# mikwieczorek/centroids-reid

Measured on AMD Instinct MI355X. Metric: train_images_per_sec, higher is better.
Workload: dtype bf16; 1 GPU; ResNet50 256x128 CTL training step: fwd+bwd, centroid-triplet + center + xent, Adam + center SGD (BASELINE configs[1]); P=16, K=4, global_batch=64, num_classes=751, parallelism=single

## Files before the change

centroids-reid_amd/csrc/conv_igemm.hip:

```cpp
#include "conv_common.hpp"
#include <type_traits>
#include "wgrad_reduce.hpp"
#include "tune.hpp"
#include <stdlib.h>

bool wgrad_make_reduce_job(const creid_conv_desc* d, int dtype, const void* ws, size_t ws_bytes, float* dw, int accumulate,
                           WRedJob& j);
int wgrad_reduce_job_launch(const WRedJob& j, hipStream_t s);
int launch_stream1x1(int M, int K, int N, const void* src, const void* wgt, void* out, float* bn_part, hipStream_t s);
int launch_stream2(int M, int K, int N, const void* src, const void* wgt, void* out, float* bn_part, const void* add_src,
                   const float* epi_scale, const float* epi_shift, int epi_relu, int bn_cap, int dtype, hipStream_t s);
int launch_conv3x3_c64(int M, int H, int Wd, const void* src, const void* wgt, void* out, float* bn_part, const float* epi_scale,
                       const float* epi_shift, int epi_relu, int dtype, hipStream_t s);
int launch_igemm_pp(const IGemmGeom& g, const void* src, const void* wgt, void* out, const void* add_src, float* bn_part,
                    int variant, int dtype, hipStream_t s);

__device__ __attribute__((aligned(128))) unsigned g_zero_page[32];

template <int BN>
__global__ __launch_bounds__(256, BN == 128 ? 1 : 2) void igemm_bf16_kernel(IGemmGeom g, const unsigned short* __restrict__ src,
                                                         const unsigned short* __restrict__ wgt,
                                                         unsigned short* __restrict__ out,
                                                         const unsigned short* __restrict__ add_src,
                                                         float* __restrict__ bn_part, int tiles_n) {
  constexpr int BK = 64, TNW = BN / 64, NB = BN / 32;
  constexpr int CP = BN + 8;
  constexpr int LDS_ELEMS = (128 * BK + BN * BK) > (128 * CP) ? (128 * BK + BN * BK) : (128 * CP);
  __shared__ __attribute__((aligned(16))) unsigned short smem[LDS_ELEMS];
  unsigned short* As = smem;
  unsigned short* Bs = smem + 128 * BK;
  const int tid = threadIdx.x, lane = tid & 63, wave = tid >> 6;
  const int wm = wave >> 1, wn = wave & 1;
  const int bid = xcd_remap(blockIdx.x, gridDim.x);
  const int tile_m = bid / tiles_n, tile_n = bid % tiles_n;
  const int row0 = tile_m * 128, col0 = tile_n * BN;
  const int span_mask = (1 << g.log2span) - 1;
  const bool tap_uniform = g.log2span >= 6;

  const int lrow = tid >> 3, lch = tid & 7;
  int oy[4], ox[4], bpix[4], soff[4];
  bool vm[4];
#pragma unroll
  for (int i = 0; i < 4; ++i) {
    const int r = lrow + 32 * i, m = row0 + r;
    vm[i] = m < g.M;
    const int mm = vm[i] ? m : 0;
    int b, rem;
    fast_divmod(mm, g.OH * g.OW, g.inv_ohow, b, rem);
    fast_divmod(rem, g.OW, g.inv_ow, oy[i], ox[i]);
    bpix[i] = b * g.SH * g.SW;
    soff[i] = r * BK + ((lch ^ ((r >> 1) & 7)) << 3);
  }
  const unsigned short* wp[NB];
#pragma unroll
  for (int i = 0; i < NB; ++i) wp[i] = wgt + (int64_t)(col0 + lrow + 32 * i) * g.K + 8 * lch;

  const unsigned short* aptr[4];
  int amul[4];
  int cur_tap = -1;
  const unsigned short* zpage = reinterpret_cast<const unsigned short*>(g_zero_page) + 8 * lch;
  auto set_tap = [&](int tap) {
    const int r = tap / g.kw, s = tap - r * g.kw;
#pragma unroll
    for (int i = 0; i < 4; ++i) {
      int iy, ix;
      const bool ok = vm[i] && igemm_src_pixel(g, oy[i], ox[i], r, s, iy, ix);
      aptr[i] = ok ? src + (int64_t)(bpix[i] + iy * g.SW + ix) * g.pitch + 8 * lch : zpage;
      amul[i] = ok ? 1 : 0;
    }
  };
  typedef unsigned u32x4 __attribute__((ext_vector_type(4)));
  struct Stage { u32x4 a0, a1, a2, a3, b0, b1, b2, b3; };
  Stage st0, st1, st2;
  const u32x4 zero4 = {0u, 0u, 0u, 0u};
#define IGEMM_LDA(I_, DST, C_) DST = *reinterpret_cast<const u32x4*>(aptr[I_] + (C_) * amul[I_])
#define IGEMM_LDA_G(I_, DST, R_, S_, C_)                                                                \
  do {                                                                                                  \
    int iy, ix;                                                                                         \
    if (vm[I_] && igemm_src_pixel(g, oy[I_], ox[I_], R_, S_, iy, ix))                                   \
      DST = *reinterpret_cast<const u32x4*>(src + (int64_t)(bpix[I_] + iy * g.SW + ix) * g.pitch + (C_)); \
    else                                                                                                \
      DST = zero4;                                                                                      \
  } while (0)
#define IGEMM_GLOAD(T_, ST)                                                                             \
  do {                                                                                                  \
    const int t_ = (T_);                                                                                \
    if (tap_uniform) {                                                                                  \
      const int tap_ = (t_ * BK) >> g.log2span;                                                         \
      if (tap_ != cur_tap) { set_tap(tap_); cur_tap = tap_; }                                           \
      const int c_ = (t_ * BK) & span_mask;                                                             \
      IGEMM_LDA(0, ST.a0, c_); IGEMM_LDA(1, ST.a1, c_); IGEMM_LDA(2, ST.a2, c_); IGEMM_LDA(3, ST.a3, c_); \
    } else {                                                                                            \
      const int kk_ = t_ * BK + 8 * lch;                                                                \
      const int tap_ = kk_ >> g.log2span, c_ = kk_ & span_mask;                                         \
      const int r_ = tap_ / g.kw, s_ = tap_ - r_ * g.kw;                                                \
      IGEMM_LDA_G(0, ST.a0, r_, s_, c_); IGEMM_LDA_G(1, ST.a1, r_, s_, c_);                             \
      IGEMM_LDA_G(2, ST.a2, r_, s_, c_); IGEMM_LDA_G(3, ST.a3, r_, s_, c_);                             \
    }                                                                                                   \
    ST.b0 = *reinterpret_cast<const u32x4*>(wp[0] + t_ * BK);                                           \
    ST.b1 = *reinterpret_cast<const u32x4*>(wp[1] + t_ * BK);                                           \
    if constexpr (NB == 4) {                                                                            \
      ST.b2 = *reinterpret_cast<const u32x4*>(wp[2] + t_ * BK);                                         \
      ST.b3 = *reinterpret_cast<const u32x4*>(wp[3] + t_ * BK);                                         \
    }                                                                                                   \
  } while (0)
#define IGEMM_LSTORE(ST)                                                                                \
  do {                                                                                                  \
    *reinterpret_cast<u32x4*>(&As[soff[0]]) = ST.a0; *reinterpret_cast<u32x4*>(&As[soff[1]]) = ST.a1;   \
    *reinterpret_cast<u32x4*>(&As[soff[2]]) = ST.a2; *reinterpret_cast<u32x4*>(&As[soff[3]]) = ST.a3;   \
    *reinterpret_cast<u32x4*>(&Bs[soff[0]]) = ST.b0; *reinterpret_cast<u32x4*>(&Bs[soff[1]]) = ST.b1;   \
    if constexpr (NB == 4) {                                                                            \
      *reinterpret_cast<u32x4*>(&Bs[soff[2]]) = ST.b2; *reinterpret_cast<u32x4*>(&Bs[soff[3]]) = ST.b3; \
    }                                                                                                   \
  } while (0)

  f32x16 acc[2][TNW];
#pragma unroll
  for (int i = 0; i < 2; ++i)
#pragma unroll
    for (int j = 0; j < TNW; ++j)
#pragma unroll
      for (int r = 0; r < 16; ++r) acc[i][j][r] = 0.f;

  const int nk = g.K / BK;
  const int l31 = lane & 31, kh = lane >> 5;
  auto compute = [&]() {
#pragma unroll
    for (int kk = 0; kk < 4; ++kk) {
      const int ch = 2 * kk + kh;
      s16x8 a[2], b[TNW];
#pragma unroll
      for (int i = 0; i < 2; ++i) {
        const int r = wm * 64 + i * 32 + l31;
        a[i] = *reinterpret_cast<const s16x8*>(&As[r * BK + ((ch ^ ((r >> 1) & 7)) << 3)]);
      }
#pragma unroll
      for (int j = 0; j < TNW; ++j) {
        const int c = wn * (BN / 2) + j * 32 + l31;
        b[j] = *reinterpret_cast<const s16x8*>(&Bs[c * BK + ((ch ^ ((c >> 1) & 7)) << 3)]);
      }
#pragma unroll
      for (int i = 0; i < 2; ++i)
#pragma unroll
        for (int j = 0; j < TNW; ++j)
          acc[i][j] = __builtin_amdgcn_mfma_f32_32x32x16_bf16(__builtin_bit_cast(bf16x8, a[i]),
                                                              __builtin_bit_cast(bf16x8, b[j]), acc[i][j], 0, 0, 0);
    }
  };
  const int last = nk - 1;
  IGEMM_GLOAD(0, st0);
  IGEMM_GLOAD(min(1, last), st1);
  IGEMM_GLOAD(min(2, last), st2);
  const int nk3 = nk - nk % 3;
  int t = 0;
  for (; t < nk3; t += 3) {
    __syncthreads();
    IGEMM_LSTORE(st0);
    __syncthreads();
    IGEMM_GLOAD(min(t + 3, last), st0);
    compute();
    __syncthreads();
    IGEMM_LSTORE(st1);
    __syncthreads();
    IGEMM_GLOAD(min(t + 4, last), st1);
    compute();
    __syncthreads();
    IGEMM_LSTORE(st2);
    __syncthreads();
    IGEMM_GLOAD(min(t + 5, last), st2);
    compute();
  }
  for (; t < nk; ++t) {
    __syncthreads();
    IGEMM_LSTORE(st0);
    __syncthreads();
    st0 = st1;
    compute();
  }
#undef IGEMM_GLOAD
#undef IGEMM_LSTORE
#undef IGEMM_LDA
#undef IGEMM_LDA_G
  __syncthreads();

  float s1v[TNW], s2v[TNW];
#pragma unroll
  for (int j = 0; j < TNW; ++j) {
    const int cl = wn * (BN / 2) + j * 32 + l31;
    float s1 = 0.f, s2 = 0.f;
#pragma unroll
    for (int i = 0; i < 2; ++i) {
#pragma unroll
      for (int r = 0; r < 16; ++r) {
        const int rl = wm * 64 + i * 32 + (r & 3) + 8 * (r >> 2) + 4 * kh;
        const float v = acc[i][j][r];
        s1 += v; s2 = fmaf(v, v, s2);
        smem[rl * CP + cl] = f32_to_bf16_bits(v);
      }
    }
    s1 += __shfl_xor(s1, 32, 64); s2 += __shfl_xor(s2, 32, 64);
    s1v[j] = s1; s2v[j] = s2;
  }
  __syncthreads();
  constexpr int CPR = BN / 8;
#pragma unroll
  for (int i = 0; i < (128 * CPR) / 256; ++i) {
    const int id = tid + 256 * i, rl = id / CPR, ch = id - rl * CPR;
    const int rr = row0 + rl;
    if (rr < g.M) {
      uint4 v = *reinterpret_cast<const uint4*>(&smem[rl * CP + ch * 8]);
      const int64_t off = (int64_t)rr * g.N + col0 + ch * 8;
      if (add_src) {
        const uint4 a = *reinterpret_cast<const uint4*>(add_src + off);
        unsigned* vw = &v.x; const unsigned* aw = &a.x;
#pragma unroll
        for (int q = 0; q < 4; ++q) {
          const float lo = __uint_as_float(vw[q] << 16) + __uint_as_float(aw[q] << 16);
          const float hi = __uint_as_float(vw[q] & 0xffff0000u) + __uint_as_float(aw[q] & 0xffff0000u);
          vw[q] = (unsigned)f32_to_bf16_bits(lo) | ((unsigned)f32_to_bf16_bits(hi) << 16);
        }
      }
      *reinterpret_cast<uint4*>(out + off) = v;
    }
  }
  if (bn_part) {
    __syncthreads();
    float* red = reinterpret_cast<float*>(smem);
#pragma unroll
    for (int j = 0; j < TNW; ++j) {
      const int cl = wn * (BN / 2) + j * 32 + l31;
      if (kh == 0) { red[(wm * 2 + 0) * BN + cl] = s1v[j]; red[(wm * 2 + 1) * BN + cl] = s2v[j]; }
    }
    __syncthreads();
    for (int i = tid; i < 2 * BN; i += 256) {
      const int which = i / BN, cl = i - which * BN;
      bn_part[((int64_t)tile_m * 2 + which) * g.N + col0 + cl] = red[(0 * 2 + which) * BN + cl] + red[(1 * 2 + which) * BN + cl];
    }
  }
}

template <int N> __device__ __forceinline__ void wait_vm() { asm volatile("s_waitcnt vmcnt(%0)" ::"n"(N) : "memory"); }

template <int BN, int NS, typename ET = Bf16T>
__global__ __launch_bounds__(256, (NS * (128 + BN) * 128 <= 80 * 1024) ? 2 : 1) void igemm_bf16_dma_kernel(IGemmGeom g, const unsigned short* __restrict__ src,
                                                                 const unsigned short* __restrict__ wgt,
                                                                 unsigned short* __restrict__ out,
                                                                 const unsigned short* __restrict__ add_src,
                                                                 float* __restrict__ bn_part, int tiles_n,
                                                                 BnRedArgs bnred) {
  constexpr int BK = 64, TNW = BN / 64, NBI = BN / 32;
  constexpr int CPT = 128 + 4;
  constexpr int TILE_A = 128 * BK, TILE_B = BN * BK, STAGE = TILE_A + TILE_B;
  constexpr int LDS_ELEMS = (NS * STAGE) > (BN * CPT) ? (NS * STAGE) : (BN * CPT);
  constexpr int LPT = 4 + NBI;
  static_assert((NS - 2) * LPT <= 63, "vmcnt is a 6-bit counter");
  __shared__ __attribute__((aligned(1024))) unsigned short smem[LDS_ELEMS];
  const int tid = threadIdx.x, lane = tid & 63, wave = tid >> 6;
  const int wm = wave >> 1, wn = wave & 1;
  const int bid = xcd_remap(blockIdx.x, gridDim.x);
  const int tile_m = bid / tiles_n, tile_n = bid % tiles_n;
  const int row0 = tile_m * 128, col0 = tile_n * BN;
  const int span_mask = (1 << g.log2span) - 1;

  const int lr8 = lane >> 3, lcp = lane & 7;
  int oy[4], ox[4], bpix[4], gch[4];
  bool vm[4];
#pragma unroll
  for (int i = 0; i < 4; ++i) {
    const int r = (i * 4 + wave) * 8 + lr8, m = row0 + r;
    vm[i] = m < g.M;
    const int mm = vm[i] ? m : 0;
    int b, rem;
    fast_divmod(mm, g.OH * g.OW, g.inv_ohow, b, rem);
    fast_divmod(rem, g.OW, g.inv_ow, oy[i], ox[i]);
    bpix[i] = b * g.SH * g.SW;
    gch[i] = (lcp ^ ((r >> 1) & 7)) << 3;
  }
  const unsigned short* wp[NBI];
#pragma unroll
  for (int i = 0; i < NBI; ++i) {
    const int r = (i * 4 + wave) * 8 + lr8;
    wp[i] = wgt + (int64_t)(col0 + r) * g.K + ((lcp ^ ((r >> 1) & 7)) << 3);
  }
  const unsigned short* aptr[4];
  int amul[4];
  int cur_tap = -1, cur_r = 0, cur_s = -1;
  const unsigned short* zpage = reinterpret_cast<const unsigned short*>(g_zero_page);
  auto set_tap = [&]() {
    if (++cur_s == g.kw) { cur_s = 0; ++cur_r; }
    const int r = cur_r, s = cur_s;
#pragma unroll
    for (int i = 0; i < 4; ++i) {
      int iy, ix;
      const bool ok = vm[i] && igemm_src_pixel(g, oy[i], ox[i], r, s, iy, ix);
      aptr[i] = ok ? src + (int64_t)(bpix[i] + iy * g.SW + ix) * g.pitch + gch[i] : zpage;
      amul[i] = ok ? 1 : 0;
    }
  };
  typedef const void __attribute__((address_space(1)))* gptr_t;
  typedef void __attribute__((address_space(3)))* lptr_t;
  const bool stem = g.log2span == 5;
  const int stem_step = 2 * g.SW * g.pitch;
  if (stem) {
#pragma unroll
    for (int i = 0; i < 4; ++i) {
      const int sc = gch[i] >> 3;
      aptr[i] = vm[i] ? src + (int64_t)(bpix[i] + (oy[i] * 2 + (sc >> 2)) * g.SW + ox[i] * 2) * g.pitch + (sc & 3) * 8 : zpage;
      amul[i] = vm[i] ? 1 : 0;
    }
  }
  auto issue = [&](int t, int buf) {
    if (!stem) {
      const int tap = (t * BK) >> g.log2span;
      if (tap != cur_tap) { set_tap(); cur_tap = tap; }
    }
    unsigned short* la = smem + buf * STAGE + wave * 512;
    unsigned short* lb = smem + buf * STAGE + TILE_A + wave * 512;
    const int a_step = stem ? stem_step : BK;
#pragma unroll
    for (int i = 0; i < 4; ++i) {
      __builtin_amdgcn_global_load_lds((gptr_t)aptr[i], (lptr_t)(la + i * 2048), 16, 0, 0);
      aptr[i] += amul[i] ? a_step : 0;
    }
#pragma unroll
    for (int i = 0; i < NBI; ++i) {
      __builtin_amdgcn_global_load_lds((gptr_t)wp[i], (lptr_t)(lb + i * 2048), 16, 0, 0);
      wp[i] += BK;
    }
  };

  f32x16 acc[2][TNW];
#pragma unroll
  for (int i = 0; i < 2; ++i)
#pragma unroll
    for (int j = 0; j < TNW; ++j)
#pragma unroll
      for (int r = 0; r < 16; ++r) acc[i][j][r] = 0.f;

  const int nk = g.K / BK;
  const int l31 = lane & 31, kh = lane >> 5;
#pragma unroll
  for (int p = 0; p < NS - 1; ++p)
    if (p < nk) issue(p, p);
  int buf = 0;
  for (int t = 0; t < nk; ++t) {
    const int younger = min(nk - 1 - t, NS - 2);
    if constexpr (NS >= 5) { if (younger == 3) wait_vm<3 * LPT>(); }
    if constexpr (NS >= 4) { if (younger == 2) wait_vm<2 * LPT>(); }
    if constexpr (NS >= 3) { if (younger == 1) wait_vm<1 * LPT>(); }
    if (younger == 0) wait_vm<0>();
    asm volatile("s_barrier" ::: "memory");
    if (t + NS - 1 < nk) issue(t + NS - 1, buf == 0 ? NS - 1 : buf - 1);
    const unsigned short* As = smem + buf * STAGE;
    buf = (buf + 1 == NS) ? 0 : buf + 1;
    const unsigned short* Bs = As + TILE_A;
    s16x8 a[4][2], b[4][TNW];
#pragma unroll
    for (int kk = 0; kk < 4; ++kk) {
      const int ch = 2 * kk + kh;
#pragma unroll
      for (int i = 0; i < 2; ++i) {
        const int r = wm * 64 + i * 32 + l31;
        a[kk][i] = *reinterpret_cast<const s16x8*>(&As[r * BK + ((ch ^ ((r >> 1) & 7)) << 3)]);
      }
#pragma unroll
      for (int j = 0; j < TNW; ++j) {
        const int c = wn * (BN / 2) + j * 32 + l31;
        b[kk][j] = *reinterpret_cast<const s16x8*>(&Bs[c * BK + ((ch ^ ((c >> 1) & 7)) << 3)]);
      }
    }
    __builtin_amdgcn_sched_barrier(0);
#pragma unroll
    for (int kk = 0; kk < 4; ++kk)
#pragma unroll
      for (int i = 0; i < 2; ++i)
#pragma unroll
        for (int j = 0; j < TNW; ++j)
          acc[i][j] = ET::mfma(a[kk][i], b[kk][j], acc[i][j]);
  }
  __syncthreads();

  constexpr int NPRE = (128 * (BN / 8)) / 256;
  constexpr int CPR = BN / 8;
  static_assert(16 % CPR == 0, "copy-out map: 8 or 16 column octets per tile row");
  const int t4 = lane & 3, q4 = (lane >> 2) & 3, g4 = lane >> 4;
  auto unit_of = [&](int i, int& rl, int& ch) {
    const int Q = (wave + 4 * i) * 16 + g4 * 4 + q4;
    ch = Q % CPR;
    rl = 4 * (Q / CPR) + t4;
  };
  uint4 pre_x[NPRE], pre_a[NPRE];
  unsigned pre_m[NPRE];
  if (bnred.x && bnred.prefetch) {
    const unsigned short* bx0 = reinterpret_cast<const unsigned short*>(bnred.x);
    const unsigned short* ba0 = reinterpret_cast<const unsigned short*>(bnred.act);
#pragma unroll
    for (int i = 0; i < NPRE; ++i) {
      int rl, ch;
      unit_of(i, rl, ch);
      const int rr = row0 + rl;
      pre_x[i] = make_uint4(0u, 0u, 0u, 0u);
      pre_a[i] = make_uint4(ET::ONE2, ET::ONE2, ET::ONE2, ET::ONE2);
      pre_m[i] = 0xffu;
      if (rr < g.M) {
        const int64_t off = (int64_t)rr * g.N + col0 + ch * 8;
        pre_x[i] = *reinterpret_cast<const uint4*>(bx0 + off);
        if (bnred.mask) pre_m[i] = bnred.mask[off >> 3];
        else if (ba0) pre_a[i] = *reinterpret_cast<const uint4*>(ba0 + off);
      }
    }
  }
  float s1v[TNW], s2v[TNW];
  if (g.epi_scale) {
    const bool relu_now = g.epi_relu && !add_src;
#pragma unroll
    for (int j = 0; j < TNW; ++j) {
      const int cl = wn * (BN / 2) + j * 32 + l31;
      const float sc = g.epi_scale[col0 + cl], sh = g.epi_shift[col0 + cl];
#pragma unroll
      for (int i = 0; i < 2; ++i) {
#pragma unroll
        for (int q = 0; q < 4; ++q) {
          const int rl = wm * 64 + i * 32 + 8 * q + 4 * kh;
          float v0 = fmaf(acc[i][j][4 * q], sc, sh), v1 = fmaf(acc[i][j][4 * q + 1], sc, sh);
          float v2 = fmaf(acc[i][j][4 * q + 2], sc, sh), v3 = fmaf(acc[i][j][4 * q + 3], sc, sh);
          if (relu_now) { v0 = fmaxf(v0, 0.f); v1 = fmaxf(v1, 0.f); v2 = fmaxf(v2, 0.f); v3 = fmaxf(v3, 0.f); }
          *reinterpret_cast<uint2*>(&smem[cl * CPT + rl]) = make_uint2(ET::pack2(v0, v1), ET::pack2(v2, v3));
        }
      }
      s1v[j] = 0.f; s2v[j] = 0.f;
    }
  } else {
#pragma unroll
  for (int j = 0; j < TNW; ++j) {
    const int cl = wn * (BN / 2) + j * 32 + l31;
    float s1 = 0.f, s2 = 0.f;
#pragma unroll
    for (int i = 0; i < 2; ++i) {
#pragma unroll
      for (int q = 0; q < 4; ++q) {
        const int rl = wm * 64 + i * 32 + 8 * q + 4 * kh;
        const float v0 = acc[i][j][4 * q], v1 = acc[i][j][4 * q + 1], v2 = acc[i][j][4 * q + 2], v3 = acc[i][j][4 * q + 3];
        s1 += v0; s2 = fmaf(v0, v0, s2);
        s1 += v1; s2 = fmaf(v1, v1, s2);
        s1 += v2; s2 = fmaf(v2, v2, s2);
        s1 += v3; s2 = fmaf(v3, v3, s2);
        *reinterpret_cast<uint2*>(&smem[cl * CPT + rl]) = make_uint2(ET::pack2(v0, v1), ET::pack2(v2, v3));
      }
    }
    s1 += __shfl_xor(s1, 32, 64); s2 += __shfl_xor(s2, 32, 64);
    s1v[j] = s1; s2v[j] = s2;
  }
  }
  __syncthreads();
  constexpr int NIT = (128 * CPR) / 256;
  u32x2 trlo[NIT], trhi[NIT];
  {
    const int sq = lane & 3, sj = (lane >> 2) & 3;
#pragma unroll
    for (int i = 0; i < NIT; ++i) {
      const int Qs = (wave + 4 * i) * 16 + g4 * 4 + sq;
      const unsigned addr = (unsigned)(uintptr_t)&smem[((Qs % CPR) * 8 + sj) * CPT + 4 * (Qs / CPR)];
      asm volatile("ds_read_b64_tr_b16 %0, %2\n\tds_read_b64_tr_b16 %1, %2 offset:%3"
                   : "=&v"(trlo[i]), "=&v"(trhi[i]) : "v"(addr), "i"(4 * CPT * 2) : "memory");
    }
    asm volatile("s_waitcnt lgkmcnt(0)" ::: "memory");
#pragma unroll
    for (int i = 0; i < NIT; ++i) asm volatile("" : "+v"(trlo[i]), "+v"(trhi[i]));
  }
  constexpr int NRG = 256 / CPR;
  const unsigned short* bx = reinterpret_cast<const unsigned short*>(bnred.x);
  const unsigned short* bact = reinterpret_cast<const unsigned short*>(bnred.act);
  float rs1[8], rs2[8], rmu[8], ris[8];
  if (bx) {
    const int c0 = col0 + ((g4 * 4 + q4) % CPR) * 8;
#pragma unroll
    for (int k = 0; k < 8; k += 4) {
      const int64_t so = bnred.tiles_per_image ? (int64_t)(tile_m / bnred.tiles_per_image) * g.N : 0;
      const float4 a = *reinterpret_cast<const float4*>(bnred.mean + so + c0 + k);
      const float4 b = *reinterpret_cast<const float4*>(bnred.invstd + so + c0 + k);
      rmu[k] = a.x; rmu[k + 1] = a.y; rmu[k + 2] = a.z; rmu[k + 3] = a.w;
      ris[k] = b.x; ris[k + 1] = b.y; ris[k + 2] = b.z; ris[k + 3] = b.w;
    }
#pragma unroll
    for (int k = 0; k < 8; ++k) { rs1[k] = 0.f; rs2[k] = 0.f; }
  }
#pragma unroll
  for (int i = 0; i < NIT; ++i) {
    int rl, ch;
    unit_of(i, rl, ch);
    const int rr = row0 + rl;
    if (rr < g.M) {
      uint4 v = make_uint4(trlo[i].x, trlo[i].y, trhi[i].x, trhi[i].y);
      const int64_t off = (int64_t)rr * g.N + col0 + ch * 8;
      if (add_src) {
        int64_t aoff = off;
        bool has = true;
        if (g.add_compact) {
          int ab, arem, ay, ax;
          fast_divmod(rr, g.OH * g.OW, g.inv_ohow, ab, arem);
          fast_divmod(arem, g.OW, g.inv_ow, ay, ax);
          has = ((ay | ax) & 1) == 0;
          aoff = (int64_t)((ab * (g.OH >> 1) + (ay >> 1)) * (g.OW >> 1) + (ax >> 1)) * g.N + col0 + ch * 8;
        }
        if (has) {
          const uint4 a = *reinterpret_cast<const uint4*>(add_src + aoff);
          const unsigned am = g.add_mask ? (unsigned)g.add_mask[aoff >> 3] : 0xffu;
          unsigned* vw = &v.x; const unsigned* aw = &a.x;
#pragma unroll
          for (int q = 0; q < 4; ++q) {
            const float alo = ((am >> (2 * q)) & 1u) ? ET::lo(aw[q]) : 0.f;
            const float ahi = ((am >> (2 * q + 1)) & 1u) ? ET::hi(aw[q]) : 0.f;
            float lo = ET::lo(vw[q]) + alo;
            float hi = ET::hi(vw[q]) + ahi;
            if (g.epi_relu) { lo = fmaxf(lo, 0.f); hi = fmaxf(hi, 0.f); }
            vw[q] = ET::pack2(lo, hi);
          }
        }
      }
      *reinterpret_cast<uint4*>(out + off) = v;
      if (bx) {
        uint4 xv = pre_x[i], av = pre_a[i];
        unsigned mb = pre_m[i];
        if (!bnred.prefetch) {
          xv = *reinterpret_cast<const uint4*>(bx + off);
          av = make_uint4(ET::ONE2, ET::ONE2, ET::ONE2, ET::ONE2);
          if (bnred.mask) mb = bnred.mask[off >> 3];
          else if (bact) av = *reinterpret_cast<const uint4*>(bact + off);
        }
        const unsigned* vw = &v.x; const unsigned* xw = &xv.x; const unsigned* aw = &av.x;
#pragma unroll
        for (int q = 0; q < 4; ++q) {
          float g0 = ET::lo(vw[q]), g1 = ET::hi(vw[q]);
          const float a0 = ET::lo(aw[q]), a1 = ET::hi(aw[q]);
          const float x0 = ET::lo(xw[q]), x1 = ET::hi(xw[q]);
          g0 = (a0 > 0.f && ((mb >> (2 * q)) & 1u)) ? g0 : 0.f; g1 = (a1 > 0.f && ((mb >> (2 * q + 1)) & 1u)) ? g1 : 0.f;
          rs1[2 * q] += g0; rs1[2 * q + 1] += g1;
          rs2[2 * q] = fmaf(g0, (x0 - rmu[2 * q]) * ris[2 * q], rs2[2 * q]);
          rs2[2 * q + 1] = fmaf(g1, (x1 - rmu[2 * q + 1]) * ris[2 * q + 1], rs2[2 * q + 1]);
        }
      }
    }
  }
  if (bx) {
    __syncthreads();
    float* red2 = reinterpret_cast<float*>(smem);
    const int cidx = g4 * 4 + q4;
    const int rg = (wave * 4 + t4) * (16 / CPR) + cidx / CPR, cb = (cidx % CPR) * 8;
#pragma unroll
    for (int k = 0; k < 8; ++k) { red2[(rg * 2 + 0) * BN + cb + k] = rs1[k]; red2[(rg * 2 + 1) * BN + cb + k] = rs2[k]; }
    __syncthreads();
    for (int i = tid; i < 2 * BN; i += 256) {
      const int which = i / BN, cl = i - which * BN;
      float a = 0.f;
#pragma unroll
      for (int q = 0; q < NRG; ++q) a += red2[(q * 2 + which) * BN + cl];
      bnred.partial[((int64_t)tile_m * 2 + which) * g.N + col0 + cl] = a;
    }
  }
  if (bn_part) {
    __syncthreads();
    float* red = reinterpret_cast<float*>(smem);
#pragma unroll
    for (int j = 0; j < TNW; ++j) {
      const int cl = wn * (BN / 2) + j * 32 + l31;
      if (kh == 0) { red[(wm * 2 + 0) * BN + cl] = s1v[j]; red[(wm * 2 + 1) * BN + cl] = s2v[j]; }
    }
    __syncthreads();
    for (int i = tid; i < 2 * BN; i += 256) {
      const int which = i / BN, cl = i - which * BN;
      bn_part[((int64_t)tile_m * 2 + which) * g.N + col0 + cl] = red[(0 * 2 + which) * BN + cl] + red[(1 * 2 + which) * BN + cl];
    }
  }
}

template <int BN, int NS, int BM = 128, typename ET = Bf16T>
__global__ __launch_bounds__(512, (BN == 64 && NS == 2 && BM == 128) ? 6 : ((NS * (BM + BN) * 128 <= 80 * 1024) ? 2 : 1)) void igemm_bf16_ws_kernel(IGemmGeom g, const unsigned short* __restrict__ src,
                                                                const unsigned short* __restrict__ wgt,
                                                                unsigned short* __restrict__ out,
                                                                const unsigned short* __restrict__ add_src,
                                                                float* __restrict__ bn_part, int tiles_n,
                                                                BnRedArgs bnred, WRedJob wred) {
  constexpr int NT = 512;
  constexpr int BK = 64, TNW = BN / 64, NBI = BN / 32;
  constexpr int MI = BM / 64, NAI = BM / 32;
  constexpr int CPT = BM + 4;
  constexpr int TILE_A = BM * BK, TILE_B = BN * BK, STAGE = TILE_A + TILE_B;
  constexpr int CPR = BN / 8, NRG = NT / CPR;
  constexpr int RED_ELEMS = NRG * 2 * BN * 2;
  constexpr int LDS0 = (NS * STAGE) > (BN * CPT) ? (NS * STAGE) : (BN * CPT);
  constexpr int LDS_ELEMS = LDS0 > RED_ELEMS ? LDS0 : RED_ELEMS;
  constexpr int LPT = NAI + NBI;
  static_assert(NS >= 2 && (NS - 2) * LPT <= 63, "ring depth");
  static_assert(BM == 128 || BM == 256, "row tile");
  __shared__ __attribute__((aligned(1024))) unsigned short smem[LDS_ELEMS];
  const int tid = threadIdx.x, lane = tid & 63, wave = tid >> 6;
  const int nred = wred.ws ? wred.nblocks : 0;
  const int ntile_wgs = (int)gridDim.x - nred;
  if ((int)blockIdx.x >= ntile_wgs) {
    wgrad_reduce_block<NT>(wred, (int)blockIdx.x - ntile_wgs, reinterpret_cast<float*>(smem));
    return;
  }
  const bool producer = wave >= 4;
  const int cw = wave & 3;
  const int wm = cw >> 1, wn = cw & 1;
  const int bid = xcd_remap((int)blockIdx.x, ntile_wgs);
  const int tile_m = bid / tiles_n, tile_n = bid % tiles_n;
  const int row0 = tile_m * BM, col0 = tile_n * BN;
  const int l31 = lane & 31, kh = lane >> 5;
  const int msub = g.M >> 2;
  const int cls = g.parity ? row0 / msub : 0, py = cls >> 1, px = cls & 1;
  const int tstep = g.parity ? 2 : 1;
  const int r0 = g.parity ? ((py + g.pad) & 1) : 0, s0 = g.parity ? ((px + g.pad) & 1) : 0;
  const int kh_taps = (g.K >> g.log2span) / g.kw;
  const int nk = g.parity ? ((kh_taps - r0 + 1) / 2) * ((g.kw - s0 + 1) / 2) * ((1 << g.log2span) / BK) : g.K / BK;
  auto pixel_of = [&](int rr) -> int {
    if (!g.parity) return rr;
    const int rem2 = rr - cls * msub;
    int b, rem, a, c;
    fast_divmod(rem2, (g.OH >> 1) * (g.OW >> 1), g.inv_ohow * 4.f, b, rem);
    fast_divmod(rem, g.OW >> 1, g.inv_ow * 2.f, a, c);
    return (b * g.OH + 2 * a + py) * g.OW + 2 * c + px;
  };

  f32x16 acc[MI][TNW];
  if (producer) {
    const int span_mask = (1 << g.log2span) - 1;
    const int lr8 = lane >> 3, lcp = lane & 7;
    int oy[NAI], ox[NAI], bpix[NAI], gch[NAI];
    bool vm[NAI];
#pragma unroll
    for (int i = 0; i < NAI; ++i) {
      const int r = (i * 4 + cw) * 8 + lr8, m = row0 + r;
      vm[i] = m < g.M;
      const int mm = vm[i] ? m : row0;
      const int pix = pixel_of(mm);
      int b, rem;
      fast_divmod(pix, g.OH * g.OW, g.inv_ohow, b, rem);
      fast_divmod(rem, g.OW, g.inv_ow, oy[i], ox[i]);
      bpix[i] = b * g.SH * g.SW;
      gch[i] = (lcp ^ ((r >> 1) & 7)) << 3;
    }
    const unsigned short* wp[NBI];
    const unsigned short* wbase[NBI];
#pragma unroll
    for (int i = 0; i < NBI; ++i) {
      const int r = (i * 4 + cw) * 8 + lr8;
      wbase[i] = wgt + (int64_t)(col0 + r) * g.K + ((lcp ^ ((r >> 1) & 7)) << 3);
      wp[i] = wbase[i];
    }
    const unsigned short* aptr[NAI];
    int amul[NAI];
    int cur_tap = -1, cur_r = r0, cur_s = s0 - tstep;
    const unsigned short* zpage = reinterpret_cast<const unsigned short*>(g_zero_page);
    typedef const void __attribute__((address_space(1)))* gptr_t;
    typedef void __attribute__((address_space(3)))* lptr_t;
    auto issue = [&](int t, int buf) {
      if (CREID_ABL_ON(g.abl, 2) && t > 0) return;
      const int tap = (t * BK) >> g.log2span;
      if (tap != cur_tap) {
        cur_tap = tap;
        cur_s += tstep;
        if (cur_s >= g.kw) { cur_s = s0; cur_r += tstep; }
        if (g.parity) {
#pragma unroll
          for (int i = 0; i < NBI; ++i) wp[i] = wbase[i] + ((cur_r * g.kw + cur_s) << g.log2span);
        }
#pragma unroll
        for (int i = 0; i < NAI; ++i) {
          int iy, ix;
          const bool ok = vm[i] && igemm_src_pixel(g, oy[i], ox[i], cur_r, cur_s, iy, ix);
          aptr[i] = ok ? src + (int64_t)(bpix[i] + iy * g.SW + ix) * g.pitch + gch[i] : zpage;
          amul[i] = ok ? 1 : 0;
        }
      }
      unsigned short* la = smem + buf * STAGE + cw * 512;
      unsigned short* lb = smem + buf * STAGE + TILE_A + cw * 512;
#pragma unroll
      for (int i = 0; i < NAI; ++i) {
        __builtin_amdgcn_global_load_lds((gptr_t)aptr[i], (lptr_t)(la + i * 2048), 16, 0, 0);
        aptr[i] += amul[i] ? BK : 0;
      }
#pragma unroll
      for (int i = 0; i < NBI; ++i) {
        __builtin_amdgcn_global_load_lds((gptr_t)wp[i], (lptr_t)(lb + i * 2048), 16, 0, 0);
        wp[i] += BK;
      }
    };
#pragma unroll
    for (int p = 0; p < NS - 1; ++p)
      if (p < nk) issue(p, p);
    int buf = 0;
    for (int t = 0; t < nk; ++t) {
      const int younger = min(nk - 1 - t, NS - 2);
      if constexpr (NS >= 5) { if (younger == 3) wait_vm<3 * LPT>(); }
      if constexpr (NS >= 4) { if (younger == 2) wait_vm<2 * LPT>(); }
      if constexpr (NS >= 3) { if (younger == 1) wait_vm<1 * LPT>(); }
      if (younger == 0) wait_vm<0>();
      asm volatile("s_barrier" ::: "memory");
      if (t + NS - 1 < nk) issue(t + NS - 1, buf == 0 ? NS - 1 : buf - 1);
      buf = (buf + 1 == NS) ? 0 : buf + 1;
    }
  } else {
#pragma unroll
    for (int i = 0; i < MI; ++i)
#pragma unroll
      for (int j = 0; j < TNW; ++j)
#pragma unroll
        for (int r = 0; r < 16; ++r) acc[i][j][r] = 0.f;
    int buf = 0;
    for (int t = 0; t < nk; ++t) {
      asm volatile("s_barrier" ::: "memory");
      const unsigned short* As = smem + buf * STAGE;
      const unsigned short* Bs = As + TILE_A;
      buf = (buf + 1 == NS) ? 0 : buf + 1;
      s16x8 a[2][MI], b[2][TNW];
      auto load_frags = [&](int kk, int sl) {
        const int ch = 2 * kk + kh;
#pragma unroll
        for (int i = 0; i < MI; ++i) {
          const int r = wm * (BM / 2) + i * 32 + l31;
          a[sl][i] = *reinterpret_cast<const s16x8*>(&As[r * BK + ((ch ^ ((r >> 1) & 7)) << 3)]);
        }
#pragma unroll
        for (int j = 0; j < TNW; ++j) {
          const int c = wn * (BN / 2) + j * 32 + l31;
          b[sl][j] = *reinterpret_cast<const s16x8*>(&Bs[c * BK + ((ch ^ ((c >> 1) & 7)) << 3)]);
        }
      };
      auto mma = [&](int sl) {
        if (CREID_ABL_ON(g.abl, 1)) return;
#pragma unroll
        for (int i = 0; i < MI; ++i)
#pragma unroll
          for (int j = 0; j < TNW; ++j)
            acc[i][j] = ET::mfma(a[sl][i], b[sl][j], acc[i][j]);
      };
      if (CREID_ABL_ON(g.abl, 4)) continue;
      load_frags(0, 0);
      __builtin_amdgcn_sched_barrier(0);
      load_frags(1, 1); mma(0);
      __builtin_amdgcn_sched_barrier(0);
      load_frags(2, 0); mma(1);
      __builtin_amdgcn_sched_barrier(0);
      load_frags(3, 1); mma(0);
      __builtin_amdgcn_sched_barrier(0);
      mma(1);
    }
  }
  __syncthreads();

  constexpr int NPRE = BM == 128 ? (128 * (BN / 8)) / 512 : 1;
  const int t4 = lane & 3, q4 = (lane >> 2) & 3, g4 = lane >> 4;
  auto unit_of = [&](int i, int& rl, int& ch) {
    const int Q = (wave + 8 * i) * 16 + g4 * 4 + q4;
    ch = Q % CPR;
    rl = 4 * (Q / CPR) + t4;
  };
  uint4 pre_x[NPRE], pre_a[NPRE];
  unsigned pre_m[NPRE];
  if (BM == 128 && bnred.x && bnred.prefetch) {
    const unsigned short* bx0 = reinterpret_cast<const unsigned short*>(bnred.x);
    const unsigned short* ba0 = reinterpret_cast<const unsigned short*>(bnred.act);
#pragma unroll
    for (int i = 0; i < NPRE; ++i) {
      int rl, ch;
      unit_of(i, rl, ch);
      const int rr = row0 + rl;
      pre_x[i] = make_uint4(0u, 0u, 0u, 0u);
      pre_a[i] = make_uint4(ET::ONE2, ET::ONE2, ET::ONE2, ET::ONE2);
      pre_m[i] = 0xffu;
      if (rr < g.M) {
        const int64_t off = (int64_t)pixel_of(rr) * g.N + col0 + ch * 8;
        pre_x[i] = *reinterpret_cast<const uint4*>(bx0 + off);
        if (bnred.mask) pre_m[i] = bnred.mask[off >> 3];
        else if (ba0) pre_a[i] = *reinterpret_cast<const uint4*>(ba0 + off);
      }
    }
  }
  float s1v[TNW], s2v[TNW];
  if (!producer && g.epi_scale) {
    const bool relu_now = g.epi_relu && !add_src;
#pragma unroll
    for (int j = 0; j < TNW; ++j) {
      const int cl = wn * (BN / 2) + j * 32 + l31;
      const float sc = g.epi_scale[col0 + cl], sh = g.epi_shift[col0 + cl];
#pragma unroll
      for (int i = 0; i < MI; ++i) {
#pragma unroll
        for (int q = 0; q < 4; ++q) {
          const int rl = wm * (BM / 2) + i * 32 + 8 * q + 4 * kh;
          float v0 = fmaf(acc[i][j][4 * q], sc, sh), v1 = fmaf(acc[i][j][4 * q + 1], sc, sh);
          float v2 = fmaf(acc[i][j][4 * q + 2], sc, sh), v3 = fmaf(acc[i][j][4 * q + 3], sc, sh);
          if (relu_now) { v0 = fmaxf(v0, 0.f); v1 = fmaxf(v1, 0.f); v2 = fmaxf(v2, 0.f); v3 = fmaxf(v3, 0.f); }
          *reinterpret_cast<uint2*>(&smem[cl * CPT + rl]) = make_uint2(ET::pack2(v0, v1), ET::pack2(v2, v3));
        }
      }
      s1v[j] = 0.f; s2v[j] = 0.f;
    }
  } else if (!producer) {
#pragma unroll
    for (int j = 0; j < TNW; ++j) {
      const int cl = wn * (BN / 2) + j * 32 + l31;
      float s1 = 0.f, s2 = 0.f;
#pragma unroll
      for (int i = 0; i < MI; ++i) {
#pragma unroll
        for (int q = 0; q < 4; ++q) {
          const int rl = wm * (BM / 2) + i * 32 + 8 * q + 4 * kh;
          const float v0 = acc[i][j][4 * q], v1 = acc[i][j][4 * q + 1], v2 = acc[i][j][4 * q + 2], v3 = acc[i][j][4 * q + 3];
          s1 += v0; s2 = fmaf(v0, v0, s2);
          s1 += v1; s2 = fmaf(v1, v1, s2);
          s1 += v2; s2 = fmaf(v2, v2, s2);
          s1 += v3; s2 = fmaf(v3, v3, s2);
          *reinterpret_cast<uint2*>(&smem[cl * CPT + rl]) = make_uint2(ET::pack2(v0, v1), ET::pack2(v2, v3));
        }
      }
      s1 += __shfl_xor(s1, 32, 64); s2 += __shfl_xor(s2, 32, 64);
      s1v[j] = s1; s2v[j] = s2;
    }
  }
  __syncthreads();
  constexpr int NIT = (BM * CPR) / NT;
  static_assert(16 % CPR == 0, "copy-out map: 8 or 16 column octets per tile row");
  u32x2 trlo[NIT], trhi[NIT];
  {
    const int sq = lane & 3, sj = (lane >> 2) & 3;
#pragma unroll
    for (int i = 0; i < NIT; ++i) {
      const int Qs = (wave + 8 * i) * 16 + g4 * 4 + sq;
      const unsigned addr = (unsigned)(uintptr_t)&smem[((Qs % CPR) * 8 + sj) * CPT + 4 * (Qs / CPR)];
      asm volatile("ds_read_b64_tr_b16 %0, %2\n\tds_read_b64_tr_b16 %1, %2 offset:%3"
                   : "=&v"(trlo[i]), "=&v"(trhi[i]) : "v"(addr), "i"(4 * CPT * 2) : "memory");
    }
  }
  const unsigned short* bx = BM == 128 ? reinterpret_cast<const unsigned short*>(bnred.x) : nullptr;
  const unsigned short* bact = reinterpret_cast<const unsigned short*>(bnred.act);
  float rs1[8], rs2[8], rmu[8], ris[8];
  if (bx) {
    const int c0 = col0 + ((g4 * 4 + q4) % CPR) * 8;
#pragma unroll
    for (int k = 0; k < 8; k += 4) {
      const int64_t so = bnred.tiles_per_image ? (int64_t)(tile_m / bnred.tiles_per_image) * g.N : 0;
      const float4 a = *reinterpret_cast<const float4*>(bnred.mean + so + c0 + k);
      const float4 b = *reinterpret_cast<const float4*>(bnred.invstd + so + c0 + k);
      rmu[k] = a.x; rmu[k + 1] = a.y; rmu[k + 2] = a.z; rmu[k + 3] = a.w;
      ris[k] = b.x; ris[k + 1] = b.y; ris[k + 2] = b.z; ris[k + 3] = b.w;
    }
#pragma unroll
    for (int k = 0; k < 8; ++k) { rs1[k] = 0.f; rs2[k] = 0.f; }
  }
  asm volatile("s_waitcnt lgkmcnt(0)" ::: "memory");
#pragma unroll
  for (int i = 0; i < NIT; ++i) asm volatile("" : "+v"(trlo[i]), "+v"(trhi[i]));
#pragma unroll
  for (int i = 0; i < NIT; ++i) {
    int rl, ch;
    unit_of(i, rl, ch);
    const int rr = row0 + rl;
    if (rr < g.M) {
      uint4 v = make_uint4(trlo[i].x, trlo[i].y, trhi[i].x, trhi[i].y);
      const int prow = pixel_of(rr);
      const int64_t off = (int64_t)prow * g.N + col0 + ch * 8;
      if (add_src) {
        int64_t aoff = off;
        bool has = true;
        if (g.add_compact) {
          int ab, arem, ay, ax;
          fast_divmod(prow, g.OH * g.OW, g.inv_ohow, ab, arem);
          fast_divmod(arem, g.OW, g.inv_ow, ay, ax);
          has = ((ay | ax) & 1) == 0;
          aoff = (int64_t)((ab * (g.OH >> 1) + (ay >> 1)) * (g.OW >> 1) + (ax >> 1)) * g.N + col0 + ch * 8;
        }
        if (has) {
          const uint4 a = *reinterpret_cast<const uint4*>(add_src + aoff);
          const unsigned am = g.add_mask ? (unsigned)g.add_mask[aoff >> 3] : 0xffu;
          unsigned* vw = &v.x; const unsigned* aw = &a.x;
#pragma unroll
          for (int q = 0; q < 4; ++q) {
            const float alo = ((am >> (2 * q)) & 1u) ? ET::lo(aw[q]) : 0.f;
            const float ahi = ((am >> (2 * q + 1)) & 1u) ? ET::hi(aw[q]) : 0.f;
            float lo = ET::lo(vw[q]) + alo;
            float hi = ET::hi(vw[q]) + ahi;
            if (g.epi_relu) { lo = fmaxf(lo, 0.f); hi = fmaxf(hi, 0.f); }
            vw[q] = ET::pack2(lo, hi);
          }
        }
      }
      if (!CREID_ABL_ON(g.abl, 8)) *reinterpret_cast<uint4*>(out + off) = v;
      if (bx) {
        uint4 xv = pre_x[i % NPRE], av = pre_a[i % NPRE];
        unsigned mb = pre_m[i % NPRE];
        if (!bnred.prefetch) {
          xv = *reinterpret_cast<const uint4*>(bx + off);
          av = make_uint4(ET::ONE2, ET::ONE2, ET::ONE2, ET::ONE2);
          if (bnred.mask) mb = bnred.mask[off >> 3];
          else if (bact) av = *reinterpret_cast<const uint4*>(bact + off);
        }
        const unsigned* vw = &v.x; const unsigned* xw = &xv.x; const unsigned* aw = &av.x;
#pragma unroll
        for (int q = 0; q < 4; ++q) {
          float g0 = ET::lo(vw[q]), g1 = ET::hi(vw[q]);
          const float a0 = ET::lo(aw[q]), a1 = ET::hi(aw[q]);
          const float x0 = ET::lo(xw[q]), x1 = ET::hi(xw[q]);
          g0 = (a0 > 0.f && ((mb >> (2 * q)) & 1u)) ? g0 : 0.f; g1 = (a1 > 0.f && ((mb >> (2 * q + 1)) & 1u)) ? g1 : 0.f;
          rs1[2 * q] += g0; rs1[2 * q + 1] += g1;
          rs2[2 * q] = fmaf(g0, (x0 - rmu[2 * q]) * ris[2 * q], rs2[2 * q]);
          rs2[2 * q + 1] = fmaf(g1, (x1 - rmu[2 * q + 1]) * ris[2 * q + 1], rs2[2 * q + 1]);
        }
      }
    }
  }
  if (bx) {
    __syncthreads();
    float* red2 = reinterpret_cast<float*>(smem);
    const int cidx = g4 * 4 + q4;
    const int rg = (wave * 4 + t4) * (16 / CPR) + cidx / CPR, cb = (cidx % CPR) * 8;
#pragma unroll
    for (int k = 0; k < 8; ++k) { red2[(rg * 2 + 0) * BN + cb + k] = rs1[k]; red2[(rg * 2 + 1) * BN + cb + k] = rs2[k]; }
    __syncthreads();
    for (int i = tid; i < 2 * BN; i += NT) {
      const int which = i / BN, cl = i - which * BN;
      float a = 0.f;
#pragma unroll 8
      for (int q = 0; q < NRG; ++q) a += red2[(q * 2 + which) * BN + cl];
      bnred.partial[((int64_t)tile_m * 2 + which) * g.N + col0 + cl] = a;
    }
  }
  if (bn_part) {
    __syncthreads();
    float* red = reinterpret_cast<float*>(smem);
    if (!producer) {
#pragma unroll
      for (int j = 0; j < TNW; ++j) {
        const int cl = wn * (BN / 2) + j * 32 + l31;
        if (kh == 0) { red[(wm * 2 + 0) * BN + cl] = s1v[j]; red[(wm * 2 + 1) * BN + cl] = s2v[j]; }
      }
    }
    __syncthreads();
    for (int i = tid; i < 2 * BN; i += NT) {
      const int which = i / BN, cl = i - which * BN;
      if constexpr (BM == 128) {
        bn_part[((int64_t)tile_m * 2 + which) * g.N + col0 + cl] = red[(0 * 2 + which) * BN + cl] + red[(1 * 2 + which) * BN + cl];
      } else {
        bn_part[((int64_t)(tile_m * 2 + 0) * 2 + which) * g.N + col0 + cl] = red[(0 * 2 + which) * BN + cl];
        if (row0 + 128 < g.M) bn_part[((int64_t)(tile_m * 2 + 1) * 2 + which) * g.N + col0 + cl] = red[(1 * 2 + which) * BN + cl];
      }
    }
  }
}

template <int BN>
__global__ __launch_bounds__(256) void igemm_f32_kernel(IGemmGeom g, const float* __restrict__ src,
                                                        const float* __restrict__ wgt, float* __restrict__ out,
                                                        const float* __restrict__ add_src,
                                                        float* __restrict__ bn_part, int tiles_n) {
  constexpr int BK = 16, PA = 128 * 4 + 16, PB = BN * 4 + 16, TNW = BN / 64, NB = BN / 64;
  __shared__ __attribute__((aligned(16))) float As[2][2][2][PA];
  __shared__ __attribute__((aligned(16))) float Bs[2][2][2][PB];
  const int tid = threadIdx.x, lane = tid & 63, wave = tid >> 6;
  const int wm = wave >> 1, wn = wave & 1;
  const int bid = xcd_remap(blockIdx.x, gridDim.x);
  const int tile_m = bid / tiles_n, tile_n = bid % tiles_n;
  const int row0 = tile_m * 128, col0 = tile_n * BN;
  const int span_mask = (1 << g.log2span) - 1;

  const int lrow = tid >> 2, lkc = tid & 3;
  int oy[2], ox[2], bpix[2];
  bool vm[2];
#pragma unroll
  for (int i = 0; i < 2; ++i) {
    const int m = row0 + lrow + 64 * i;
    vm[i] = m < g.M;
    const int mm = vm[i] ? m : 0;
    const int b = mm / (g.OH * g.OW), rem = mm - b * (g.OH * g.OW);
    oy[i] = rem / g.OW; ox[i] = rem - oy[i] * g.OW;
    bpix[i] = b * g.SH * g.SW;
  }
  const float* wp[NB];
#pragma unroll
  for (int i = 0; i < NB; ++i) wp[i] = wgt + (int64_t)(col0 + lrow + 64 * i) * g.K + 4 * lkc;
  float4 ra[2], rb[NB];
  unsigned amask[2] = {0u, 0u};
  auto gload = [&](int t) {
    const int kk = t * BK + 4 * lkc;
    const int tap = kk >> g.log2span, c = kk & span_mask;
    const int r = tap / g.kw, s = tap - r * g.kw;
#pragma unroll
    for (int i = 0; i < 2; ++i) {
      int iy, ix;
      const bool ok = vm[i] && igemm_src_pixel(g, oy[i], ox[i], r, s, iy, ix);
      amask[i] = ok ? 0xffffffffu : 0u;
      const int64_t off = ok ? (int64_t)(bpix[i] + iy * g.SW + ix) * g.pitch + c : 0;
      ra[i] = *reinterpret_cast<const float4*>(src + off);
    }
#pragma unroll
    for (int i = 0; i < NB; ++i) rb[i] = *reinterpret_cast<const float4*>(wp[i] + t * BK);
  };
  const int sh = lkc >> 1, so = lrow * 4 + 2 * (lkc & 1);
  auto lstore = [&](int buf) {
#pragma unroll
    for (int i = 0; i < 2; ++i) {
      auto mk = [&](float v) { return __uint_as_float(__float_as_uint(v) & amask[i]); };
      *reinterpret_cast<float2*>(&As[buf][0][sh][so + 256 * i]) = make_float2(mk(ra[i].x), mk(ra[i].z));
      *reinterpret_cast<float2*>(&As[buf][1][sh][so + 256 * i]) = make_float2(mk(ra[i].y), mk(ra[i].w));
    }
#pragma unroll
    for (int i = 0; i < NB; ++i) {
      *reinterpret_cast<float2*>(&Bs[buf][0][sh][so + 256 * i]) = make_float2(rb[i].x, rb[i].z);
      *reinterpret_cast<float2*>(&Bs[buf][1][sh][so + 256 * i]) = make_float2(rb[i].y, rb[i].w);
    }
  };
  f32x16 acc[2][TNW];
#pragma unroll
  for (int i = 0; i < 2; ++i)
#pragma unroll
    for (int j = 0; j < TNW; ++j)
#pragma unroll
      for (int r = 0; r < 16; ++r) acc[i][j][r] = 0.f;
  const int nk = g.K / BK;
  const int l31 = lane & 31, kh = lane >> 5;
  const int fa = (wm * 64 + l31) * 4, fb = (wn * (BN / 2) + l31) * 4;
  float4 a0[2], b0[TNW], a1[2], b1[TNW];
  auto frag = [&](int buf, int half, float4 (&a)[2], float4 (&b)[TNW]) {
#pragma unroll
    for (int i = 0; i < 2; ++i) a[i] = *reinterpret_cast<const float4*>(&As[buf][kh][half][fa + 128 * i]);
#pragma unroll
    for (int j = 0; j < TNW; ++j) b[j] = *reinterpret_cast<const float4*>(&Bs[buf][kh][half][fb + 128 * j]);
  };
  auto mma = [&](const float4 (&a)[2], const float4 (&b)[TNW]) {
#pragma unroll
    for (int s4 = 0; s4 < 4; ++s4) {
      float av[2], bv[TNW];
#pragma unroll
      for (int i = 0; i < 2; ++i) { const float c4[4] = {a[i].x, a[i].y, a[i].z, a[i].w}; av[i] = c4[s4]; }
#pragma unroll
      for (int j = 0; j < TNW; ++j) { const float c4[4] = {b[j].x, b[j].y, b[j].z, b[j].w}; bv[j] = c4[s4]; }
#pragma unroll
      for (int i = 0; i < 2; ++i)
#pragma unroll
        for (int j = 0; j < TNW; ++j) acc[i][j] = __builtin_amdgcn_mfma_f32_32x32x2f32(av[i], bv[j], acc[i][j], 0, 0, 0);
    }
  };
  gload(0);
  lstore(0);
  __syncthreads();
  gload(nk > 1 ? 1 : 0);
  frag(0, 0, a0, b0);
  for (int t = 0; t + 1 < nk; ++t) {
    const int buf = t & 1;
    __builtin_amdgcn_sched_barrier(0);
// ... 400 lines not shown
```

Baseline: 10890 images/s.

## Hoist next k-tile fragment loads before last MFMA and use inline-asm LDS DMA

Restructures the consumer loop of the warp-specialized DMA implicit-GEMM conv kernel. The first LDS fragment load of the next k-tile is now issued right after the barrier and before the final MFMA batch of the current tile, so LDS latency overlaps matrix math instead of stalling at the top of each iteration. The producer's global_load_lds builtin is replaced by inline asm that sets M0 from a readfirstlane-uniform LDS address, to avoid per-issue address setup overhead. Risks include subtle synchronization errors from the manual barrier and lgkmcnt placement, and the hand-written M0 handling.

```diff
diff --git a/centroids-reid_amd/csrc/conv_igemm.hip b/centroids-reid_amd/csrc/conv_igemm.hip
--- a/centroids-reid_amd/csrc/conv_igemm.hip
+++ b/centroids-reid_amd/csrc/conv_igemm.hip
@@ -240,6 +240,9 @@
 }
 
 template <int N> __device__ __forceinline__ void wait_vm() { asm volatile("s_waitcnt vmcnt(%0)" ::"n"(N) : "memory"); }
+__device__ __forceinline__ void glds16_asm(const unsigned short* gsrc, unsigned lds_addr) {
+  asm volatile("s_mov_b32 m0, %1\n\ts_nop 0\n\tglobal_load_lds_dwordx4 %0, off" ::"v"(gsrc), "s"(lds_addr) : "memory");
+}
 
 template <int BN, int NS, typename ET = Bf16T>
 __global__ __launch_bounds__(256, (NS * (128 + BN) * 128 <= 80 * 1024) ? 2 : 1) void igemm_bf16_dma_kernel(IGemmGeom g, const unsigned short* __restrict__ src,
@@ -653,8 +656,6 @@
     int amul[NAI];
     int cur_tap = -1, cur_r = r0, cur_s = s0 - tstep;
     const unsigned short* zpage = reinterpret_cast<const unsigned short*>(g_zero_page);
-    typedef const void __attribute__((address_space(1)))* gptr_t;
-    typedef void __attribute__((address_space(3)))* lptr_t;
     auto issue = [&](int t, int buf) {
       if (CREID_ABL_ON(g.abl, 2) && t > 0) return;
       const int tap = (t * BK) >> g.log2span;
@@ -674,16 +675,16 @@
           amul[i] = ok ? 1 : 0;
         }
       }
-      unsigned short* la = smem + buf * STAGE + cw * 512;
-      unsigned short* lb = smem + buf * STAGE + TILE_A + cw * 512;
+      const unsigned la = __builtin_amdgcn_readfirstlane((unsigned)(uintptr_t)(smem + buf * STAGE + cw * 512));
+      const unsigned lb = la + TILE_A * 2;
 #pragma unroll
       for (int i = 0; i < NAI; ++i) {
-        __builtin_amdgcn_global_load_lds((gptr_t)aptr[i], (lptr_t)(la + i * 2048), 16, 0, 0);
+        glds16_asm(aptr[i], la + i * 4096);
         aptr[i] += amul[i] ? BK : 0;
       }
 #pragma unroll
       for (int i = 0; i < NBI; ++i) {
-        __builtin_amdgcn_global_load_lds((gptr_t)wp[i], (lptr_t)(lb + i * 2048), 16, 0, 0);
+        glds16_asm(wp[i], lb + i * 4096);
         wp[i] += BK;
       }
     };
@@ -708,45 +709,67 @@
       for (int j = 0; j < TNW; ++j)
 #pragma unroll
         for (int r = 0; r < 16; ++r) acc[i][j][r] = 0.f;
-    int buf = 0;
-    for (int t = 0; t < nk; ++t) {
-      asm volatile("s_barrier" ::: "memory");
-      const unsigned short* As = smem + buf * STAGE;
+    s16x8 a[2][MI], b[2][TNW];
+    auto load_frags = [&](const unsigned short* As, int kk, int sl) {
       const unsigned short* Bs = As + TILE_A;
-      buf = (buf + 1 == NS) ? 0 : buf + 1;
-      s16x8 a[2][MI], b[2][TNW];
-      auto load_frags = [&](int kk, int sl) {
-        const int ch = 2 * kk + kh;
-#pragma unroll
-        for (int i = 0; i < MI; ++i) {
-          const int r = wm * (BM / 2) + i * 32 + l31;
-          a[sl][i] = *reinterpret_cast<const s16x8*>(&As[r * BK + ((ch ^ ((r >> 1) & 7)) << 3)]);
-        }
-#pragma unroll
-        for (int j = 0; j < TNW; ++j) {
-          const int c = wn * (BN / 2) + j * 32 + l31;
-          b[sl][j] = *reinterpret_cast<const s16x8*>(&Bs[c * BK + ((ch ^ ((c >> 1) & 7)) << 3)]);
-        }
-      };
-      auto mma = [&](int sl) {
-        if (CREID_ABL_ON(g.abl, 1)) return;
-#pragma unroll
-        for (int i = 0; i < MI; ++i)
-#pragma unroll
-          for (int j = 0; j < TNW; ++j)
-            acc[i][j] = ET::mfma(a[sl][i], b[sl][j], acc[i][j]);
-      };
-      if (CREID_ABL_ON(g.abl, 4)) continue;
-      load_frags(0, 0);
+      const int ch = 2 * kk + kh;
+#pragma unroll
+      for (int i = 0; i < MI; ++i) {
+        const int r = wm * (BM / 2) + i * 32 + l31;
+        a[sl][i] = *reinterpret_cast<const s16x8*>(&As[r * BK + ((ch ^ ((r >> 1) & 7)) << 3)]);
+      }
+#pragma unroll
+      for (int j = 0; j < TNW; ++j) {
+        const int c = wn * (BN / 2) + j * 32 + l31;
+        b[sl][j] = *reinterpret_cast<const s16x8*>(&Bs[c * BK + ((ch ^ ((c >> 1) & 7)) << 3)]);
+      }
+    };
+    auto mma = [&](int sl) {
+      if (CREID_ABL_ON(g.abl, 1)) return;
+#pragma unroll
+      for (int i = 0; i < MI; ++i)
+#pragma unroll
+        for (int j = 0; j < TNW; ++j)
+          acc[i][j] = ET::mfma(a[sl][i], b[sl][j], acc[i][j]);
+    };
+    const bool abl_skip = CREID_ABL_ON(g.abl, 4);
+    auto ktile = [&](const unsigned short* As, bool more, const unsigned short* An) {
+      if (abl_skip) {
+        if (more) asm volatile("s_barrier" ::: "memory");
+        return;
+      }
       __builtin_amdgcn_sched_barrier(0);
-      load_frags(1, 1); mma(0);
+      load_frags(As, 1, 1);
       __builtin_amdgcn_sched_barrier(0);
-      load_frags(2, 0); mma(1);
+      mma(0);
       __builtin_amdgcn_sched_barrier(0);
-      load_frags(3, 1); mma(0);
+      load_frags(As, 2, 0);
       __builtin_amdgcn_sched_barrier(0);
       mma(1);
-    }
+      __builtin_amdgcn_sched_barrier(0);
+      load_frags(As, 3, 1);
+      __builtin_amdgcn_sched_barrier(0);
+      mma(0);
+      __builtin_amdgcn_sched_barrier(0);
+      if (more) {
+        asm volatile("s_waitcnt lgkmcnt(0)\n\ts_barrier" ::: "memory");
+        load_frags(An, 0, 0);
+        __builtin_amdgcn_sched_barrier(0);
+      }
+      mma(1);
+    };
+    __builtin_amdgcn_s_waitcnt(0xC07F);
+    if (nk > 0) {
+      asm volatile("s_barrier" ::: "memory");
+      if (!abl_skip) load_frags(smem, 0, 0);
+    }
+    int buf = 0;
+    for (int t = 0; t + 1 < nk; ++t) {
+      const unsigned short* As = smem + buf * STAGE;
+      buf = (buf + 1 == NS) ? 0 : buf + 1;
+      ktile(As, true, smem + buf * STAGE);
+    }
+    if (nk > 0) ktile(smem + buf * STAGE, false, nullptr);
   }
   __syncthreads();
 
```

Measured after the change: 10930 images/s (median of 6 runs). No clear change (+0.4%).
